# scroll-tech/zkvm-prover

Measured on AMD Instinct MI355X. Metric: chunk STARK proofs/sec (2^22-row trace), higher is better.
Workload: dtype u32; 1 GPU; full STARK proof: 2^22 x 300 degree-3 AIR + 2^22 x 2 Fibonacci AIR, blow-up 2, 100 queries, PoW 16+16 (SURVEY.md 8(d) cfg #4); proof_bytes=1128348, resident_key_bytes_per_pipeline=13503716096, inflight_per_gpu=3, parallelism=3 independent proof(s) in flight per GPU (one HIP stream each)

## Files before the change

### zkvm-prover_amd/csrc/poseidon2.hpp

```cpp
#pragma once
#include "babybear.hpp"

namespace zk {

struct Poseidon2Consts {
    static constexpr uint32_t RC[141] = {
#include "poseidon2_rc.inc"
    };
};

struct Poseidon2Diag {
    static constexpr uint32_t INV_2_8 = (1u << 24);
    static constexpr uint32_t INV_4 = (1u << 30);
    static constexpr uint32_t INV_8 = (1u << 29);
    static constexpr uint32_t INV_16 = (1u << 28);
    static constexpr uint32_t INV_2_27 = (1u << 5);
};

ZK_HD uint32_t mdouble(uint32_t x) { return red_2p(x << 1); }
template <int K>
ZK_HD uint32_t mdiv_pow2(uint32_t x) {
    const uint32_t m = (0u - x) & ((1u << K) - 1u);
    const uint64_t t = (uint64_t)m * P + x;
    return (uint32_t)(t >> K);
}
ZK_HD uint32_t mhalve(uint32_t x) { return (x & 1u) ? ((x >> 1) + ((P + 1u) >> 1)) : (x >> 1); }

ZK_HD uint32_t sbox7_rcs(uint32_t s, uint32_t rcs) {
    const int32_t x = (int32_t)(s + rcs);
    const int32_t x2 = smml(x, x), x3 = smml(x2, x), x4 = smml(x2, x2);
    return canon_signed(smml(x3, x4));
}
ZK_HD uint32_t sbox7_rc(uint32_t s, uint32_t rc) { return sbox7_rcs(s, rc - P); }
ZK_HD uint32_t sbox7(uint32_t x) {
    uint32_t x2 = mmul_lazy(x, x);
    uint32_t x3 = mmul_lazy(x2, x);
    uint32_t x4 = red_2p(mmul_lazy(x2, x2));
    return red_2p(mmul_lazy(x3, x4));
}

ZK_HD void p2_external_linear(uint32_t s[16]) {
#pragma unroll
    for (int b = 0; b < 16; b += 4) {
        uint32_t x0 = s[b], x1 = s[b + 1], x2 = s[b + 2], x3 = s[b + 3];
        uint32_t t01 = madd(x0, x1), t23 = madd(x2, x3);
        uint32_t t0123 = madd(t01, t23);
        uint32_t t01123 = madd(t0123, x1), t01233 = madd(t0123, x3);
        s[b + 3] = madd(madd(t01233, x0), x0);
        s[b + 1] = madd(madd(t01123, x2), x2);
        s[b + 0] = madd(t01123, t01);
        s[b + 2] = madd(t01233, t23);
    }
#pragma unroll
    for (int k = 0; k < 4; k++) {
        uint32_t sum = madd(madd(s[k], s[4 + k]), madd(s[8 + k], s[12 + k]));
#pragma unroll
        for (int b = 0; b < 16; b += 4) s[b + k] = madd(s[b + k], sum);
    }
}

ZK_HD void p2_internal_linear(uint32_t s[16]) {
    uint32_t sum = 0;
#ifdef ZK_P2_MODULAR_SUM
    {
        uint32_t a0 = madd(s[0], s[1]), a1 = madd(s[2], s[3]), a2 = madd(s[4], s[5]), a3 = madd(s[6], s[7]);
        uint32_t a4 = madd(s[8], s[9]), a5 = madd(s[10], s[11]), a6 = madd(s[12], s[13]), a7 = madd(s[14], s[15]);
        sum = madd(madd(madd(a0, a1), madd(a2, a3)), madd(madd(a4, a5), madd(a6, a7)));
    }
#else
    {
        const uint32_t a0 = s[0] + s[1], a1 = s[2] + s[3], a2 = s[4] + s[5], a3 = s[6] + s[7];
        const uint32_t a4 = s[8] + s[9], a5 = s[10] + s[11], a6 = s[12] + s[13], a7 = s[14] + s[15];
        const uint64_t t = (uint64_t)a0 + a1 + a2 + a3 + a4 + a5 + a6 + a7;
        const uint64_t x = (uint64_t)(uint32_t)(t >> 32) * 0x0FFFFFFEu + (uint32_t)t;
        const uint32_t y = (uint32_t)x + ((uint32_t)(x >> 32) ? 0x0FFFFFFEu : 0u);
        sum = red_2p(red_2p(y));
    }
#endif
    uint32_t d;
    s[0] = msub(sum, mdouble(s[0]));
    s[1] = madd(sum, s[1]);
    s[2] = madd(madd(sum, s[2]), s[2]);
    s[3] = madd(sum, mhalve(s[3]));
    d = madd(sum, s[4]); s[4] = madd(madd(d, s[4]), s[4]);
    s[5] = madd(sum, mdouble(mdouble(s[5])));
    s[6] = msub(sum, mhalve(s[6]));
    d = mdouble(s[7]); s[7] = msub(sum, madd(d, s[7]));
    s[8] = msub(sum, mdouble(mdouble(s[8])));
    s[9] = madd(sum, mdiv_pow2<8>(s[9]));
    s[10] = madd(sum, mdiv_pow2<2>(s[10]));
    s[11] = madd(sum, mdiv_pow2<3>(s[11]));
    s[12] = madd(sum, mdiv_pow2<27>(s[12]));
    s[13] = msub(sum, mdiv_pow2<8>(s[13]));
    s[14] = msub(sum, mdiv_pow2<4>(s[14]));
    s[15] = msub(sum, mdiv_pow2<27>(s[15]));
}

ZK_HD void poseidon2_permute(uint32_t s[16]) {
    p2_external_linear(s);
#pragma unroll
    for (int r = 0; r < 4; r++) {
#pragma unroll
        for (int i = 0; i < 16; i++) s[i] = sbox7_rc(s[i], Poseidon2Consts::RC[r * 16 + i]);
        p2_external_linear(s);
    }
#pragma unroll
    for (int r = 0; r < 13; r++) {
        s[0] = sbox7_rc(s[0], Poseidon2Consts::RC[64 + r]);
        p2_internal_linear(s);
    }
#pragma unroll
    for (int r = 0; r < 4; r++) {
#pragma unroll
        for (int i = 0; i < 16; i++) s[i] = sbox7_rc(s[i], Poseidon2Consts::RC[77 + r * 16 + i]);
        p2_external_linear(s);
    }
}

#if !defined(__HIP_DEVICE_COMPILE__) && defined(__x86_64__) && !defined(ZK_NO_HOST_AVX512)
#define ZK_HAVE_HOST_AVX512 1
void poseidon2_permute_avx512(uint32_t s[16]);
void poseidon2_permute16_avx512(uint32_t* t);
inline void poseidon2_permute16_host(uint32_t* t) {
    static const bool fast = __builtin_cpu_supports("avx512f") && __builtin_cpu_supports("avx512dq");
    if (fast) return poseidon2_permute16_avx512(t);
    for (int k = 0; k < 16; k++) {
        uint32_t s[16];
        for (int w = 0; w < 16; w++) s[w] = t[16 * w + k];
        poseidon2_permute(s);
        for (int w = 0; w < 16; w++) t[16 * w + k] = s[w];
    }
}
inline void poseidon2_permute_host(uint32_t s[16]) {
    static const bool fast = __builtin_cpu_supports("avx512f") && __builtin_cpu_supports("avx512dq");
    if (fast) poseidon2_permute_avx512(s);
    else poseidon2_permute(s);
}
#else
inline void poseidon2_permute_host(uint32_t s[16]) { poseidon2_permute(s); }
inline void poseidon2_permute16_host(uint32_t* t) {
    for (int k = 0; k < 16; k++) {
        uint32_t s[16];
        for (int w = 0; w < 16; w++) s[w] = t[16 * w + k];
        poseidon2_permute(s);
        for (int w = 0; w < 16; w++) t[16 * w + k] = s[w];
    }
}
#endif
#if defined(__HIP_DEVICE_COMPILE__)
#define ZK_P2_PERMUTE_HERE(s) poseidon2_permute(s)
#else
#define ZK_P2_PERMUTE_HERE(s) poseidon2_permute_host(s)
#endif

ZK_HD void p2_hash_slice(const uint32_t* in, size_t len, uint32_t out[8]) {
    uint32_t s[16];
    for (int i = 0; i < 16; i++) s[i] = 0;
    size_t i = 0;
    while (i < len) {
        size_t n = len - i < 8 ? len - i : 8;
        for (size_t k = 0; k < n; k++) s[k] = in[i + k];
        ZK_P2_PERMUTE_HERE(s);
        i += n;
    }
    for (int k = 0; k < 8; k++) out[k] = s[k];
}
ZK_HD void p2_compress(const uint32_t l[8], const uint32_t r[8], uint32_t out[8]) {
    uint32_t s[16];
    for (int k = 0; k < 8; k++) {
        s[k] = l[k];
        s[8 + k] = r[k];
    }
    ZK_P2_PERMUTE_HERE(s);
    for (int k = 0; k < 8; k++) out[k] = s[k];
}

}
```

### zkvm-prover_amd/csrc/poseidon2_coop.hpp

```cpp
#pragma once
#include "poseidon2.hpp"

namespace zk {

#if defined(__HIPCC__)
__device__ const uint32_t POSEIDON2_DIAG_DEV[16] = {
    P - 0x1ffffffcu , 0x0ffffffeu , 0x1ffffffcu , 0x07ffffffu ,
    0x2ffffffau , 0x3ffffff8u , P - 0x07ffffffu , P - 0x2ffffffau ,
    P - 0x3ffffff8u , 1u << 24 , 1u << 30 , 1u << 29 ,
    1u << 5 , P - (1u << 24), P - (1u << 28) , P - (1u << 5)};

static __constant__ const uint32_t POSEIDON2_RC_CONST[144] = {
#include "poseidon2_rc.inc"
};
struct Poseidon2RcShifted {
    uint32_t v[144];
};
constexpr Poseidon2RcShifted poseidon2_rc_shifted() {
    Poseidon2RcShifted t{};
    for (int i = 0; i < 77; i++) t.v[i] = Poseidon2Consts::RC[i] - P;
    for (int i = 0; i < 64; i++) t.v[80 + i] = Poseidon2Consts::RC[77 + i] - P;
    return t;
}
static __constant__ const Poseidon2RcShifted POSEIDON2_RCS_CONST = poseidon2_rc_shifted();
__device__ const Poseidon2RcShifted POSEIDON2_RCS_DEV = poseidon2_rc_shifted();
__device__ __forceinline__ void poseidon2_permute_rolled(uint32_t (&s)[16]) {
    typedef const __attribute__((address_space(4))) uint32_t* cptr;
    cptr rc = (cptr)POSEIDON2_RCS_CONST.v;
    p2_external_linear(s);
#pragma unroll 1
    for (int r = 0; r < 4; r++) {
#pragma unroll
        for (int i = 0; i < 16; i++) s[i] = sbox7_rcs(s[i], rc[r * 16 + i]);
        p2_external_linear(s);
    }
#pragma unroll 1
    for (int r = 0; r < 13; r++) {
        s[0] = sbox7_rcs(s[0], rc[64 + r]);
        p2_internal_linear(s);
    }
#pragma unroll 1
    for (int r = 0; r < 4; r++) {
#pragma unroll
        for (int i = 0; i < 16; i++) s[i] = sbox7_rcs(s[i], rc[80 + r * 16 + i]);
        p2_external_linear(s);
    }
}

template <int CTRL>
__device__ __forceinline__ uint32_t dpp(uint32_t v) {
    return (uint32_t)__builtin_amdgcn_update_dpp(0, (int)v, CTRL, 0xf, 0xf, false);
}
#define ZK_QROT1 0x39
#define ZK_QROT2 0x4E
#define ZK_QROT3 0x93
#define ZK_ROR(n) (0x120 + (n))

__device__ __forceinline__ uint32_t coop_external_linear(uint32_t x) {
    const uint32_t r1 = dpp<ZK_QROT1>(x), r2 = dpp<ZK_QROT2>(x), r3 = dpp<ZK_QROT3>(x);
    const uint32_t t = madd(madd(x, r1), madd(r2, r3));
    const uint32_t y = madd(madd(t, x), mdouble(r1));
    uint32_t s = madd(y, dpp<ZK_ROR(8)>(y));
    s = madd(s, dpp<ZK_ROR(4)>(s));
    return madd(y, s);
}
__device__ __forceinline__ uint32_t coop_sum16(uint32_t x) {
    uint32_t s = madd(x, dpp<ZK_ROR(8)>(x));
    s = madd(s, dpp<ZK_ROR(4)>(s));
    s = madd(s, dpp<ZK_ROR(2)>(s));
    return madd(s, dpp<ZK_ROR(1)>(s));
}
__device__ __forceinline__ uint32_t coop_permute(uint32_t x, unsigned lane) {
    x = coop_external_linear(x);
#pragma unroll 1
    for (int r = 0; r < 4; r++) x = coop_external_linear(sbox7_rcs(x, POSEIDON2_RCS_DEV.v[r * 16 + lane]));
    const uint32_t d = POSEIDON2_DIAG_DEV[lane];
#pragma unroll 1
    for (int r = 0; r < 13; r++) {
        const uint32_t sb = sbox7_rcs(x, POSEIDON2_RCS_DEV.v[64 + r]);
        x = lane == 0 ? sb : x;
        x = madd(mmul(x, d), coop_sum16(x));
    }
#pragma unroll 1
    for (int r = 0; r < 4; r++) x = coop_external_linear(sbox7_rcs(x, POSEIDON2_RCS_DEV.v[80 + r * 16 + lane]));
    return x;
}
struct CoopConsts {
    uint32_t ext[8], in[13], diag;
};
__device__ __forceinline__ CoopConsts coop_load_consts(unsigned lane) {
    CoopConsts c;
#pragma unroll
    for (int r = 0; r < 4; r++) c.ext[r] = POSEIDON2_RCS_DEV.v[r * 16 + lane], c.ext[4 + r] = POSEIDON2_RCS_DEV.v[80 + r * 16 + lane];
#pragma unroll
    for (int r = 0; r < 13; r++) c.in[r] = POSEIDON2_RCS_DEV.v[64 + r];
    c.diag = POSEIDON2_DIAG_DEV[lane];
    return c;
}
__device__ __forceinline__ uint32_t coop_permute_regs(uint32_t x, unsigned lane, const CoopConsts& c) {
    x = coop_external_linear(x);
#pragma unroll
    for (int r = 0; r < 4; r++) x = coop_external_linear(sbox7_rcs(x, c.ext[r]));
#pragma unroll
    for (int r = 0; r < 13; r++) {
        const uint32_t sb = sbox7_rcs(x, c.in[r]);
        x = lane == 0 ? sb : x;
        x = madd(mmul(x, c.diag), coop_sum16(x));
    }
#pragma unroll
    for (int r = 0; r < 4; r++) x = coop_external_linear(sbox7_rcs(x, c.ext[4 + r]));
    return x;
}
#endif

}
```

Baseline: 13.04 proofs/s.

## Defer Poseidon2 internal-round linear layers via precomputed diagonal-power weights

Replaces the 13 sequential internal Poseidon2 rounds in the rolled GPU permutation with an algebraically equivalent formulation. Each round's sum is computed as a 64-bit multiply-accumulate over the original state and earlier sums, using a constexpr table of diagonal powers, and the state lanes 1..15 are reconstructed once at the end. This cuts the per-round updates of all 16 lanes and the serial chain of modular adds, at the cost of more 64-bit multiplies, a larger constant table and fully unrolled code that may raise register pressure. The old round-wise path stays behind ZK_P2_ROUNDWISE.

```diff
diff --git a/zkvm-prover_amd/csrc/poseidon2.hpp b/zkvm-prover_amd/csrc/poseidon2.hpp
--- a/zkvm-prover_amd/csrc/poseidon2.hpp
+++ b/zkvm-prover_amd/csrc/poseidon2.hpp
@@ -15,6 +15,9 @@
     static constexpr uint32_t INV_8 = (1u << 29);
     static constexpr uint32_t INV_16 = (1u << 28);
     static constexpr uint32_t INV_2_27 = (1u << 5);
+    static constexpr uint32_t MONTY[16] = {
+        P - 0x1ffffffcu, 0x0ffffffeu, 0x1ffffffcu, 0x07ffffffu, 0x2ffffffau, 0x3ffffff8u, P - 0x07ffffffu, P - 0x2ffffffau,
+        P - 0x3ffffff8u, INV_2_8,     INV_4,       INV_8,       INV_2_27,    P - INV_2_8, P - INV_16,      P - INV_2_27};
 };
 
 ZK_HD uint32_t mdouble(uint32_t x) { return red_2p(x << 1); }
@@ -96,6 +99,102 @@
     s[15] = msub(sum, mdiv_pow2<27>(s[15]));
 }
 
+constexpr int P2D_FINAL_OFF = 13 * 16 + 78, P2D_WORDS = P2D_FINAL_OFF + 15 * 14;
+struct Poseidon2Deferred {
+    uint32_t v[P2D_WORDS];
+};
+constexpr uint32_t p2d_mulmod(uint32_t a, uint32_t b) { return (uint32_t)((uint64_t)a * b % P); }
+constexpr Poseidon2Deferred poseidon2_deferred_table() {
+    uint32_t rinv = 1, b = MONTY_ONE;
+    for (uint32_t e = P - 2; e; e >>= 1) {
+        if (e & 1) rinv = p2d_mulmod(rinv, b);
+        b = p2d_mulmod(b, b);
+    }
+    uint32_t pw[16][14] = {}, a[13] = {};
+    for (int i = 1; i < 16; i++) {
+        pw[i][0] = MONTY_ONE;
+        for (int j = 1; j < 14; j++) pw[i][j] = p2d_mulmod(p2d_mulmod(pw[i][j - 1], Poseidon2Diag::MONTY[i]), rinv);
+    }
+    for (int j = 0; j < 13; j++)
+        for (int i = 1; i < 16; i++) a[j] = (uint32_t)(((uint64_t)a[j] + pw[i][j]) % P);
+    Poseidon2Deferred t{};
+    for (int r = 0; r < 13; r++) {
+        const int o = r * 16 + r * (r - 1) / 2;
+        t.v[o] = Poseidon2Consts::RC[64 + r] - P;
+        for (int i = 1; i < 16; i++) t.v[o + i] = pw[i][r];
+        for (int k = 0; k < r; k++) t.v[o + 16 + k] = a[r - 1 - k];
+    }
+    for (int i = 1; i < 16; i++)
+        for (int k = 0; k < 14; k++) t.v[P2D_FINAL_OFF + 14 * (i - 1) + k] = pw[i][13 - k];
+    return t;
+}
+struct Poseidon2DeferredConsts {
+    static constexpr Poseidon2Deferred T = poseidon2_deferred_table();
+};
+
+ZK_HD uint64_t p2d_fold(uint64_t t) {
+    t = (uint64_t)(uint32_t)(t >> 32) * MONTY_ONE + (uint32_t)t;
+#if defined(__HIP_DEVICE_COMPILE__)
+    asm("" : "+v"(t));
+#endif
+    return t;
+}
+ZK_HD uint32_t p2d_reduce(uint64_t t) {
+    t = p2d_fold(t);
+    const uint32_t m = (uint32_t)t * MONTY_NEG_MU;
+    return red_2p((uint32_t)((t + (uint64_t)m * P) >> 32));
+}
+#define ZK_P2D_MAC(x, wk)                      \
+    do {                                       \
+        if (n == 4) t = p2d_fold(t), n = 0;    \
+        t += (uint64_t)(x) * (wk);             \
+        n++;                                   \
+    } while (0)
+template <class W>
+ZK_HD void p2_internal_rounds_deferred(uint32_t (&s)[16], W w) {
+    uint32_t sm[13];
+#pragma unroll
+    for (int r = 0; r < 13; r++) {
+        const int o = r * 16 + r * (r - 1) / 2;
+        uint64_t t = 0;
+        int n = 0;
+#pragma unroll
+        for (int i = 1; i < 16; i++) ZK_P2D_MAC(s[i], w[o + i]);
+#pragma unroll
+        for (int k = 0; k < r; k++) ZK_P2D_MAC(sm[k], w[o + 16 + k]);
+        const uint32_t y = sbox7_rcs(s[0], w[o]);
+        ZK_P2D_MAC(y, MONTY_ONE);
+        sm[r] = p2d_reduce(t);
+        s[0] = msub(sm[r], mdouble(y));
+    }
+#pragma unroll
+    for (int i = 1; i < 16; i++) {
+        const int o = P2D_FINAL_OFF + 14 * (i - 1);
+        uint64_t t = (uint64_t)s[i] * w[o];
+        int n = 1;
+#pragma unroll
+        for (int k = 0; k < 13; k++) ZK_P2D_MAC(sm[k], w[o + 1 + k]);
+        s[i] = p2d_reduce(t);
+    }
+}
+#undef ZK_P2D_MAC
+ZK_HD void poseidon2_permute_deferred(uint32_t (&s)[16]) {
+    p2_external_linear(s);
+#pragma unroll
+    for (int r = 0; r < 4; r++) {
+#pragma unroll
+        for (int i = 0; i < 16; i++) s[i] = sbox7_rc(s[i], Poseidon2Consts::RC[r * 16 + i]);
+        p2_external_linear(s);
+    }
+    p2_internal_rounds_deferred(s, Poseidon2DeferredConsts::T.v);
+#pragma unroll
+    for (int r = 0; r < 4; r++) {
+#pragma unroll
+        for (int i = 0; i < 16; i++) s[i] = sbox7_rc(s[i], Poseidon2Consts::RC[77 + r * 16 + i]);
+        p2_external_linear(s);
+    }
+}
+
 ZK_HD void poseidon2_permute(uint32_t s[16]) {
     p2_external_linear(s);
 #pragma unroll
diff --git a/zkvm-prover_amd/csrc/poseidon2_coop.hpp b/zkvm-prover_amd/csrc/poseidon2_coop.hpp
--- a/zkvm-prover_amd/csrc/poseidon2_coop.hpp
+++ b/zkvm-prover_amd/csrc/poseidon2_coop.hpp
@@ -24,6 +24,7 @@
 }
 static __constant__ const Poseidon2RcShifted POSEIDON2_RCS_CONST = poseidon2_rc_shifted();
 __device__ const Poseidon2RcShifted POSEIDON2_RCS_DEV = poseidon2_rc_shifted();
+static __constant__ const Poseidon2Deferred POSEIDON2_DEFERRED_CONST = poseidon2_deferred_table();
 __device__ __forceinline__ void poseidon2_permute_rolled(uint32_t (&s)[16]) {
     typedef const __attribute__((address_space(4))) uint32_t* cptr;
     cptr rc = (cptr)POSEIDON2_RCS_CONST.v;
@@ -34,11 +35,17 @@
         for (int i = 0; i < 16; i++) s[i] = sbox7_rcs(s[i], rc[r * 16 + i]);
         p2_external_linear(s);
     }
+#ifdef ZK_P2_ROUNDWISE
 #pragma unroll 1
     for (int r = 0; r < 13; r++) {
         s[0] = sbox7_rcs(s[0], rc[64 + r]);
         p2_internal_linear(s);
     }
+#else
+    cptr w = (cptr)POSEIDON2_DEFERRED_CONST.v;
+    asm("" : "+s"(w));
+    p2_internal_rounds_deferred(s, w);
+#endif
 #pragma unroll 1
     for (int r = 0; r < 4; r++) {
 #pragma unroll
```

After: 13.91 proofs/s, median of 6. 6.7% higher.
